# keith2018/TinyGPT

Hardware: AMD Instinct MI355X
Metric: decode tokens/sec (and % HBM roofline), Llama-3.2-1B bf16 batch=1, 1 GPU (higher is better)
Workload: dtype bf16; 1 GPU; Llama-3.2-1B bf16, batch 1 per GPU: 2048-token prefill then greedy decode (one step = one token, context 2054..3411); replicas=1, params=1235814400, graph=True

## Files before the change

tinygpt_amd/csrc/ctx.h:

```cpp
#pragma once
#include <hip/hip_runtime.h>

#include <algorithm>
#include <cmath>
#include <cstdarg>
#include <cstdio>
#include <cstdlib>
#include <cstring>
#include <string>
#include <vector>

#include "../../include/tgx.h"
#include "kernels/common.h"
#include "kv_pool.h"
#include "dev_mem.h"

using tgx::bf16_t;
typedef unsigned char ebyte;

namespace tgx { struct SampScratch; struct LpRecord; struct LpRow; }

constexpr int MAX_TICKET_EVENTS = 64;
constexpr int HOST_RING = 256;

struct PackedMat {
  unsigned char* P = nullptr;
  tgx::u32x4* rec = nullptr;
  long long row_bytes = 0;
  unsigned int base2 = 0;
  int ks = 0;
  int max_row_esc = 0;
  long long n_esc = 0;
};

struct LayerW {
  ebyte *in_norm = nullptr, *post_norm = nullptr;
  ebyte *wqkv = nullptr, *bqkv = nullptr, *wo = nullptr, *wgu = nullptr, *wdown = nullptr;
  PackedMat pgu, pdown;
  ebyte *q_norm = nullptr, *k_norm = nullptr;
  bool q_norm_ok = false, k_norm_ok = false;
  int merged_filled = 0;
  bool in_norm_ok = false, post_norm_ok = false, wo_ok = false, wdown_ok = false;
  ebyte *in_norm_b = nullptr, *post_norm_b = nullptr, *bo = nullptr, *bfc = nullptr, *bdown = nullptr;
  int gpt2_filled = 0;
};

struct RowState {
  float *x = nullptr, *q = nullptr, *attn = nullptr, *h = nullptr;
  float* k_raw = nullptr;
  float* logits = nullptr;
  float* probs = nullptr;
  float* part_val = nullptr;
  int* part_idx = nullptr;
  float* attn_part = nullptr;
  int *tok = nullptr, *pos = nullptr;
  long long* prompt = nullptr;
  ebyte *kcache = nullptr, *vcache = nullptr;
  const int* tbl = nullptr;
};

struct RowHost {
  int64_t past = 0;
  bool tok = false;
  bool idle = false;
  bool nologits = false;
  char fin = 0;
  int64_t lp_count = 0;
  bool probs_ok = false; tgx_sampler_cfg probs_cfg{};
  bool probs_proc = false;
  int auto_id = -1;
  void restart(int64_t len, bool idle_, char fin_) { past = len; tok = nologits = false; idle = idle_; fin = fin_; }
};

struct Tune {
  int ks = 1;
  int bpc = 4;
};

struct Profiler {
  bool on = false;
  hipEvent_t ev[2 * 8] = {};
  int64_t launches[TGX_KERNEL_COUNT] = {};
  double ms[TGX_KERNEL_COUNT] = {};
};

struct QkvEpi { bf16_t *q_hi = nullptr, *q_lo = nullptr, *k = nullptr, *v = nullptr; int past = 0; const int* tbl = nullptr; };

struct ScoreCall {
  int top_n = 0, n_score = 0;
  const long long* ids = nullptr;
  void* host = nullptr; size_t host_bytes = 0;
};

struct EmbedCall {
  static constexpr int SLICE = 32;
  int pool = 0, normalize = 0, dims = 0;
  int n = 0;
  int cur = 0;
  std::vector<int> tab;
  int slices = 0;
  float* host_out = nullptr;
  int np(int t) const { return tab[(size_t)t * 4 + 1]; }
};

namespace tgx { struct RgSeq; struct RgItem; struct MixItem; }
struct RaggedPass {
  int n = 0, M = 0, longest = 0;
  const int *rows = nullptr, *lens = nullptr, *first = nullptr;
  const long long* ids = nullptr;
  const tgx::RgSeq* seq = nullptr;
  const int* tok_seq = nullptr;
  const tgx::RgItem* items = nullptr;
  int n_items = 0;
  const int* past = nullptr;
  int ext_ns = 0;
  const tgx::MixItem *mix_split = nullptr, *mix_merge = nullptr;
  int n_mix_split = 0, n_mix_merge = 0, mix_slots = 0;
};

inline void* hip_dev_alloc(size_t bytes) { void* p = nullptr; return hipMalloc(&p, bytes) == hipSuccess ? p : nullptr; }
inline void hip_dev_free(void* p) { (void)hipFree(p); }
struct tgx_ctx {
  tgx_model_desc d{};
  DevMem mem{hip_dev_alloc, hip_dev_free};
  int device = 0;
  int num_cus = 256;
  hipStream_t stream = nullptr;
  std::string err;
  bool finalized = false;

  int dt = tgx::DT_BF16;
  size_t esz = 2;
  ebyte *embed = nullptr, *lm_head = nullptr, *final_norm = nullptr;
  ebyte *wpe = nullptr, *final_norm_b = nullptr;
  bool embed_ok = false, lm_head_ok = false, final_norm_ok = false, wpe_ok = false, final_norm_b_ok = false;
  bool gpt2 = false;
  std::vector<LayerW> L;
  int weights_packed = 1, packed_classes = 4, packed_matrices = 0, packed_fallbacks = 0, packed_max_row_esc = 0;
  PackedMat plm;
  float *rope_cos = nullptr, *rope_sin = nullptr;
  std::vector<RowState> rows;
  float *slab_x = nullptr, *slab_q = nullptr, *slab_kraw = nullptr, *slab_attn = nullptr, *slab_h = nullptr, *slab_logits = nullptr;
  float *slab_probs = nullptr, *slab_part_val = nullptr, *slab_attn_part = nullptr;
  int *slab_part_idx = nullptr, *slab_tok = nullptr, *slab_pos = nullptr;
  long long* slab_prompt = nullptr;
  ebyte *slab_k = nullptr, *slab_v = nullptr;
  size_t kv_row_elems = 0, attn_part_row = 0;
  RowState chunk[4];
  float *ch_x = nullptr, *ch_q = nullptr, *ch_kraw = nullptr, *ch_attn = nullptr, *ch_h = nullptr, *ch_part = nullptr;
  int* ch_pos = nullptr;

  int64_t past = 0;
  std::vector<RowHost> row_host;
  tgx::RowReq* row_req = nullptr;
  std::vector<tgx::RowReq> row_req_host;
  int row_union = -1;
  int batch = 0;
  bool have_logits = false, have_token = false;

  int* step = nullptr;
  int* step_done = nullptr;
  int* tok_log = nullptr;
  int log_cap = 0;
  int* host_ring = nullptr;
  int* host_ring_dev = nullptr;
  int64_t steps_issued = 0;
  hipEvent_t ticket_ev[MAX_TICKET_EVENTS] = {};
  int32_t last_sampled0 = -1;

  hipGraphExec_t step_graph = nullptr;
  hipGraphExec_t multi_graph = nullptr;
  struct GraphSet { hipGraphExec_t step = nullptr, multi = nullptr; int batch = 0; tgx_sampler_cfg cfg{}; int rows = -1; bool direct = false, mfma = false, nw4 = false; unsigned long long used = 0; };
  GraphSet graph_cache[6];
  unsigned long long graph_clock = 0;
  int graph_cur = -1;
  bool mirror_to_host = true;
  int graph_steps = 16;
  unsigned long long* seed_dev = nullptr;
  unsigned long long seed_on_dev = 0;
  bool seed_valid = false;
  tgx::SampScratch* samp_scratch = nullptr;
  unsigned long long* samp_list_comp = nullptr;
  float* samp_list_v = nullptr;
  bool have_probs = false;
  bool use_graph = true;

  Tune tune[TGX_KERNEL_COUNT];
  int lm_grid = 0, attn_nsplit = 1, attn_nsplit_opt = 0;
  int ws_rows = 0;
  float *ws_x = nullptr, *ws_out = nullptr;
  bf16_t *ws_ah = nullptr, *ws_al = nullptr;
  bf16_t* ws_al2 = nullptr;
  bf16_t *ws_qh = nullptr, *ws_ql = nullptr;
  bf16_t *ws_hh = nullptr, *ws_hl = nullptr;
  float* ws_part = nullptr; size_t ws_part_bytes = 0;
  bool poisoned = false;
  const char* launch_fault = nullptr;
  int* ws_pos = nullptr;
  float* ws_ssq = nullptr;
  int gemm_splitk = 1;
  int wide_n_min = 2;
  QkvEpi qkv_epi;
  int attn_dma = 1;
  int attn_ksplit = 1;
  int qk_fuse = 1;
  int prefill_skinny_hidden_max_wide = 2048;
  int prefill_skinny_rows = 128;
  int prefill_skinny_hidden_max = 8192;
  int skinny_dma = 1;
  int skinny_dma_rows = 1;
  int skinny_dma_oproj = 2;
  int skinny_dma_qkv = 2;
  int skinny_dma_nbw = 0;
  int decode_step_rows = 128;
  int prefill_skinny = 1;
  int skinny_wgs = 256;
  int skinny_gu_split = 0;
  int skinny_cfg_mid = 0;
  int skinny_cfg_force = -1;
  int decode_mfma_min = 3;
  bool prefill_mfma = true;
  int prefill_min_rows = 4;
  int prefill_f32_min_rows = 16;
  int gemm_tm = 0;
  int gemm_dma = 15 | (1 << 4) | (2 << 8);
  int wide_8k_max = 8;
  int debug_attn = 0;
  int attn_gmax = 0;
  int attn_direct_nw4 = 0;
  bool attn_nw4 = false;
  int attn_raw_fuse = 2;
  int attn_batch_nw8 = 1;
  int attn_batch_la = 0;
  int attn_batch_mfma = 17;
  int attn_direct_g = 1;
  int attn_direct_max = 384;
  bool attn_direct = false;
  int skinny_terms = 1;
  int skinny_ksplit = 1;
  int defer_min_rows = 129;
  int defer_reduce = 1;
  int attn_mfma_min = -1;
  bool attn_mfma = false;
  int debug_gemv = 0;
  int debug_skip = 0;
  int prof_same_layer = 0;
  int oproj_sliced = 1;
  int act16 = 0, act16_kernels = 1;
  int prefill_terms_rows = 16;
  int wide_8k_eff = 76;
  int skinny_terms_above = 2;
  int qkv_nosplit = 1;
  int splitk_8k = 1;
  bf16_t* ws_zero = nullptr;
  int oproj_fused = 1, attn_fused_max = 640, attn_fused_nw4 = 384;
  int kv_budget_tokens = 0;
  bool kv_paged = false;
  KvPool kv;
  int* kv_tbl = nullptr;
  long long* slab_acc = nullptr;
  unsigned char* rg_buf = nullptr; size_t rg_bytes = 0;
  float *rg_x = nullptr, *rg_logits = nullptr, *rg_part_val = nullptr; int* rg_part_idx = nullptr;
  int extend_attn_splits = -1;
  int extend_attn_min64 = 512, extend_attn_min128 = 1024;
  float* ext_part = nullptr; size_t ext_part_bytes = 0;
  enum { VERIFY_ROWS = TGX_MAX_DRAFT + 1 };
  float *vf_x = nullptr, *vf_logits = nullptr, *vf_part_val = nullptr; int *vf_part_idx = nullptr, *vf_rec = nullptr;
  int vf_pass_rows = 0;
  tgx::SampScratch* vs_scratch = nullptr;
  unsigned long long* vs_list_comp = nullptr;
  float* vs_list_v = nullptr;
  int* vs_draws = nullptr;
  enum { VERIFY_POSITIONS = TGX_MAX_VERIFY_POSITIONS };
  float *vj_x = nullptr, *vj_logits = nullptr, *vj_part_val = nullptr; int *vj_part_idx = nullptr, *vj_rec = nullptr, *vj_draws = nullptr;
  unsigned char* vj_args = nullptr;
  std::vector<unsigned char> vj_args_host;
  bool vf_pass_joint = false;
  int verify_last_form = 0, verify_last_splits = 0;
  int advance_attn_tiles = 16, advance_last_form = 0, advance_last_tiles = 0;
  float* mix_part = nullptr; size_t mix_part_bytes = 0;
  tgx::LpRecord* lp_ring = nullptr;
  tgx::LpRow* lp_rows = nullptr;
  float* lp_tile_max = nullptr;
  double* lp_tile_sum = nullptr;
  unsigned long long* lp_tile_keys = nullptr;
  int score_rows = 2048, score_vocab_chunk = 16384, score_last_form = 0;
  float* sc_logits = nullptr; size_t sc_logits_bytes = 0;
  unsigned char* sc_part = nullptr; size_t sc_part_bytes = 0;
  int sc_part_rows = 0;
  unsigned char* sc_out = nullptr; size_t sc_out_bytes = 0;
  unsigned char* em_buf = nullptr; size_t em_bytes = 0;
// ... 140 lines not shown
```

tinygpt_amd/csrc/decode.hip:

```cpp
#include "ctx.h"
#include "kernels/attn_decode.h"
#include "kernels/gemv.h"
#include "kernels/gemv_packed.h"
#include "kernels/oproj_sliced.h"
#include "kernels/verify.h"

int gemv_grid(const tgx_ctx* c, int units, int ks, int bpc) {
  const int upb = 4 / ks;
  const int want = (units + upb - 1) / upb;
  const int cap = c->num_cus * bpc;
  return want < cap ? want : cap;
}

static int gemv_nx(int K, int ks) { return ((K / 8) + ks * 64 - 1) / (ks * 64); }

static int gemv_auto_ks(int K, int want) {
  int ks = want;
  while (ks < 4 && gemv_nx(K, ks) > 8) ks *= 2;
  return ks;
}

static tgx::GemvArgs gemv_row(const tgx_ctx* c, tgx::GemvArgs a, int r) {
  a.x += (size_t)r * a.x_stride;
  if (a.out) a.out += (size_t)r * a.out_stride;
  if (a.q_out) a.q_out += (size_t)r * a.q_stride;
  if (a.k_raw) a.k_raw += (size_t)r * a.kraw_stride;
  if (a.k_cache) a.k_cache = (ebyte*)a.k_cache + (size_t)r * a.kv_stride * c->esz;
  if (a.v_cache) a.v_cache = (ebyte*)a.v_cache + (size_t)r * a.kv_stride * c->esz;
  if (a.pos) a.pos += r;
  if (a.blk_tbl) a.blk_tbl += (size_t)r * a.tbl_stride;
  if (a.logits) a.logits += (size_t)r * a.logits_stride;
  if (a.part_val) a.part_val += (size_t)r * a.part_stride;
  if (a.part_idx) a.part_idx += (size_t)r * a.part_stride;
  return a;
}

template <int DT, int PRO, int EPI, int NX>
static void launch_gemv_nx(tgx_ctx* c, const tgx::GemvArgs& a, int grid, int R) {
  const dim3 g(grid), b(256);
  if (R == 4) { hipLaunchKernelGGL((tgx::gemv_kernel<DT, PRO, EPI, NX, 4>), g, b, 0, c->stream, a); return; }
  if (R == 2) { hipLaunchKernelGGL((tgx::gemv_kernel<DT, PRO, EPI, NX, 2>), g, b, 0, c->stream, a); return; }
  if constexpr (DT != tgx::DT_F32 && ((PRO == tgx::PRO_RMSNORM && EPI == tgx::EPI_SILU_MUL) || (PRO == tgx::PRO_PLAIN && EPI == tgx::EPI_RESIDUAL))) {
    if (R == 1 && (a.x_acc || a.res_acc)) { hipLaunchKernelGGL((tgx::gemv_kernel<DT, PRO, EPI, NX, 1, true>), g, b, a.x_acc ? (size_t)a.K * 4 : 0, c->stream, a); return; }
  }
  for (int r = 0; r < R; r++) hipLaunchKernelGGL((tgx::gemv_kernel<DT, PRO, EPI, NX, 1>), g, b, 0, c->stream, gemv_row(c, a, r));
}

template <int PRO, int EPI, int NX>
static void launch_gemv_packed_nx(tgx_ctx* c, const tgx::GemvPackedArgs& p, int grid) {
  const dim3 g(grid), b(256);
  if constexpr (EPI != tgx::EPI_LOGITS) {
    if (p.g.x_acc || p.g.res_acc) { hipLaunchKernelGGL((tgx::gemv_packed_kernel<PRO, EPI, NX, true>), g, b, p.g.x_acc ? (size_t)p.g.K * 4 : 0, c->stream, p); return; }
  }
  hipLaunchKernelGGL((tgx::gemv_packed_kernel<PRO, EPI, NX, false>), g, b, 0, c->stream, p);
}

template <int PRO, int EPI>
static void launch_gemv_packed(tgx_ctx* c, const tgx::GemvArgs& a, const PackedMat& pk, int grid, int nx) {
  tgx::GemvPackedArgs p{};
  p.g = a; p.P = pk.P; p.rec = pk.rec; p.row_bytes = pk.row_bytes; p.base2 = pk.base2;
  switch (nx) {
    case 1: launch_gemv_packed_nx<PRO, EPI, 1>(c, p, grid); break;
    case 2: launch_gemv_packed_nx<PRO, EPI, 2>(c, p, grid); break;
    case 3: launch_gemv_packed_nx<PRO, EPI, 3>(c, p, grid); break;
    case 4: launch_gemv_packed_nx<PRO, EPI, 4>(c, p, grid); break;
    case 5: launch_gemv_packed_nx<PRO, EPI, 5>(c, p, grid); break;
    case 6: launch_gemv_packed_nx<PRO, EPI, 6>(c, p, grid); break;
    case 7: launch_gemv_packed_nx<PRO, EPI, 7>(c, p, grid); break;
    default: launch_gemv_packed_nx<PRO, EPI, 8>(c, p, grid); break;
  }
}

static int pack_matrix(tgx_ctx* c, const ebyte* W, int N, int K, int cls, int* stat_dev, PackedMat* out) {
  const int ks = gemv_auto_ks(K, c->tune[cls].ks), nx = gemv_nx(K, ks);
  if (K % 8 || K > tgx::PACKED_K_MAX || nx > 8) return TGX_OK;
  PackedMat m;
  m.ks = ks; m.row_bytes = (long long)ks * ((nx + 3) / 4) * 3072;
  int rc;
  if ((rc = dev_alloc(c, &m.P, (size_t)N * (size_t)m.row_bytes)) || (rc = dev_alloc(c, &m.rec, (size_t)N))) { dev_free(c, &m.P); return rc; }
  HIP_OK(c, hipMemsetAsync(stat_dev, 0, 4 * sizeof(int), c->stream));
  const size_t n8 = (size_t)N * K / 8;
  hipLaunchKernelGGL(tgx::packed_maxexp_kernel, dim3((unsigned)std::min<size_t>((n8 + 255) / 256, 4096)), dim3(256), 0, c->stream, reinterpret_cast<const bf16_t*>(W), n8, stat_dev);
  tgx::PackRowsArgs a{};
  a.W = reinterpret_cast<const bf16_t*>(W); a.N = N; a.K = K; a.ks = ks; a.nx = nx; a.P = m.P; a.rec = m.rec; a.row_bytes = m.row_bytes; a.stat = stat_dev;
  hipLaunchKernelGGL(tgx::pack_rows_kernel, dim3(N), dim3(64), 0, c->stream, a);
  int stat[4] = {0, 0, 0, 0};
  HIP_OK(c, hipGetLastError());
  HIP_OK(c, hipMemcpyAsync(stat, stat_dev, sizeof(stat), hipMemcpyDeviceToHost, c->stream));
  HIP_OK(c, hipStreamSynchronize(c->stream));
  c->packed_max_row_esc = std::max(c->packed_max_row_esc, stat[3]);
  if (stat[1] > 0) {
    dev_free(c, &m.P); dev_free(c, &m.rec);
    c->packed_fallbacks++;
    return TGX_OK;
  }
  const unsigned int E0 = (unsigned int)std::max(stat[0] - 15, 0);
  m.base2 = (E0 << 7) | (E0 << 23); m.n_esc = stat[2]; m.max_row_esc = stat[3];
  *out = m;
  c->packed_matrices++;
  return TGX_OK;
}

int pack_weights(tgx_ctx* c) {
  const tgx_model_desc& d = c->d;
  if (!c->weights_packed || c->dt != tgx::DT_BF16 || c->gpt2) return TGX_OK;
  int* stat_dev = nullptr;
  int rc = dev_alloc(c, &stat_dev, 4);
  for (size_t l = 0; l < c->L.size() && !rc; l++) {
    LayerW& w = c->L[l];
    if (c->packed_classes & 1) rc = pack_matrix(c, w.wgu, 2 * d.inter, d.hidden, TGX_KERNEL_GATEUP, stat_dev, &w.pgu);
    if (!rc && (c->packed_classes & 2) && d.inter <= 16384) rc = pack_matrix(c, w.wdown, d.hidden, d.inter, TGX_KERNEL_DOWN, stat_dev, &w.pdown);
  }
  if (!rc && (c->packed_classes & 4)) rc = pack_matrix(c, d.tied ? c->embed : c->lm_head, d.vocab, d.hidden, TGX_KERNEL_LMHEAD, stat_dev, &c->plm);
  dev_free(c, &stat_dev);
  return rc;
}

template <int PRO, int EPI>
static void launch_gemv(tgx_ctx* c, tgx::GemvArgs a, int cls, int R, const PackedMat* pk = nullptr) {
  const Tune& tn = c->tune[cls];
  a.dbg = ((c->debug_gemv >> (8 + cls)) & 1) ? (c->debug_gemv & 15) : 0;
  if (!a.ldw) a.ldw = a.K;
  a.ks = gemv_auto_ks(a.K, tn.ks);
  while (R > 1 && a.ks < 4 && gemv_nx(a.K, a.ks) > 4) a.ks *= 2;
  if (R == 2 && cls == TGX_KERNEL_GATEUP && a.ks == 1 && gemv_nx(a.K, 1) == 4) a.ks = 2;
  const int grid = (EPI == tgx::EPI_LOGITS) ? c->lm_grid : gemv_grid(c, a.units, a.ks, tn.bpc);
  const int nx = gemv_nx(a.K, a.ks);
  if constexpr ((PRO == tgx::PRO_RMSNORM && (EPI == tgx::EPI_SILU_MUL || EPI == tgx::EPI_LOGITS)) || (PRO == tgx::PRO_PLAIN && EPI == tgx::EPI_RESIDUAL)) {
    if (pk && pk->P && R == 1 && pk->ks == a.ks && a.ldw == a.K && !a.dbg) { launch_gemv_packed<PRO, EPI>(c, a, *pk, grid, nx); return; }
  }
  if constexpr (PRO == tgx::PRO_LAYERNORM || EPI == tgx::EPI_GELU) {
    TGX_DT_SWITCH(c->dt, switch (nx) {
      case 1: launch_gemv_nx<DT, PRO, EPI, 1>(c, a, grid, R); break;
      case 2: launch_gemv_nx<DT, PRO, EPI, 2>(c, a, grid, R); break;
      case 3: launch_gemv_nx<DT, PRO, EPI, 3>(c, a, grid, R); break;
      default: launch_gemv_nx<DT, PRO, EPI, 4>(c, a, grid, R); break;
    })
  } else {
    TGX_DT_SWITCH(c->dt, switch (nx) {
      case 1: launch_gemv_nx<DT, PRO, EPI, 1>(c, a, grid, R); break;
      case 2: launch_gemv_nx<DT, PRO, EPI, 2>(c, a, grid, R); break;
      case 3: launch_gemv_nx<DT, PRO, EPI, 3>(c, a, grid, R); break;
      case 4: launch_gemv_nx<DT, PRO, EPI, 4>(c, a, grid, R); break;
      case 5: launch_gemv_nx<DT, PRO, EPI, 5>(c, a, grid, R); break;
      case 6: launch_gemv_nx<DT, PRO, EPI, 6>(c, a, grid, R); break;
      case 7: launch_gemv_nx<DT, PRO, EPI, 7>(c, a, grid, R); break;
      default: launch_gemv_nx<DT, PRO, EPI, 8>(c, a, grid, R); break;
    })
  }
}

static void fill_strides(const tgx_ctx* c, tgx::GemvArgs& a) {
  const tgx_model_desc& d = c->d;
  a.x_stride = 0; a.out_stride = 0;
  a.q_stride = (long long)d.heads * d.head_dim; a.kraw_stride = (long long)d.kv_heads * d.head_dim;
  a.kv_stride = (long long)c->kv_row_elems; a.logits_stride = d.vocab; a.part_stride = c->lm_grid;
  a.act16 = c->act16;
}

static bool qk_fused(const tgx_ctx* c, long long kv_stride) { return c->d.qk_norm && c->d.head_dim == 128 && kv_stride != 0 && c->qk_fuse; }

bool oproj_sliced_ok(const tgx_ctx* c, int R, long long kv_stride) {
  const tgx_model_desc& d = c->d;
  if (!c->oproj_sliced || R != 1 || kv_stride == 0 || c->attn_direct || c->attn_mfma || c->gpt2 || c->dt == tgx::DT_F32 || !c->slab_acc) return false;
  if (d.head_dim != 64 || d.qk_norm || d.inter > 16384 || c->attn_nsplit > 32) return false;
  if (d.hidden > tgx::XACC_HIDDEN_MAX) return false;
  const int qd = d.heads * d.head_dim;
  if (qd % 256 == 0) return d.hidden % tgx::oproj_sliced_rows<32>() == 0;
  return qd % 128 == 0 && d.hidden % tgx::oproj_sliced_rows<16>() == 0;
}

bool oproj_fused_capable(const tgx_ctx* c) {
  const tgx_model_desc& d = c->d;
  if (!c->oproj_fused || c->gpt2 || c->dt == tgx::DT_F32 || !c->slab_acc) return false;
  return d.head_dim == 64 && !d.qk_norm && d.inter <= 16384 && d.hidden % 8 == 0 && d.hidden <= tgx::XACC_HIDDEN_MAX;
}
bool oproj_fused_ok(const tgx_ctx* c, int R, long long kv_stride) {
  return R == 1 && c->batch == 1 && kv_stride != 0 && c->attn_direct && oproj_fused_capable(c);
}
static bool resid_fixed(const tgx_ctx* c, int R, long long kv_stride) { return oproj_sliced_ok(c, R, kv_stride) || oproj_fused_ok(c, R, kv_stride); }

int launch_layer_kernel(tgx_ctx* c, RowState* rv, int R, int l, int cls, float* resid, long long kv_stride) {
  const tgx_model_desc& d = c->d;
  RowState& r = rv[0];
  const int H = d.hidden, I = d.inter, hd = d.head_dim, qd = d.heads * hd, kvd = d.kv_heads * hd;
  const size_t kv_layer = (c->kv_paged ? (size_t)c->kv.n_blocks() * d.kv_heads * tgx::KV_BLOCK : (size_t)d.kv_heads * d.max_ctx) * hd * c->esz;
  const long long kvs = c->kv_paged ? 0 : kv_stride, tbs = (c->kv_paged && kv_stride != 0) ? c->kv.tbl_stride() : 0;
  const LayerW& w = c->L[(size_t)l];
  switch (cls) {
    case TGX_KERNEL_QKV: {
      tgx::GemvArgs a{};
      fill_strides(c, a);
      a.W = w.wqkv; a.bias = w.bqkv; a.x = r.x; a.x_stride = H; a.norm_w = w.in_norm; a.eps = d.norm_eps;
      a.N = qd + 2 * kvd; a.K = H; a.units = a.N / 2;
      a.q_out = r.q; a.k_cache = r.kcache + (size_t)l * kv_layer; a.v_cache = r.vcache + (size_t)l * kv_layer; a.kv_stride = kvs;
      a.blk_tbl = r.tbl; a.tbl_stride = tbs;
      a.rope_cos = c->rope_cos; a.rope_sin = c->rope_sin; a.pos = r.pos;
      a.heads = d.heads; a.kv_heads = d.kv_heads; a.hd = hd; a.max_ctx = d.max_ctx;
      a.raw_qk = d.qk_norm ? 1 : 0; a.k_raw = r.k_raw;
      if (c->gpt2) {
        a.norm_b = w.in_norm_b;
        launch_gemv<tgx::PRO_LAYERNORM, tgx::EPI_QKV_ROPE>(c, a, TGX_KERNEL_QKV, R);
        break;
      }
      launch_gemv<tgx::PRO_RMSNORM, tgx::EPI_QKV_ROPE>(c, a, TGX_KERNEL_QKV, R);
      if (d.qk_norm && !qk_fused(c, kv_stride)) {
        tgx::QkNormArgs n{};
        n.q = r.q; n.k_raw = r.k_raw; n.k_cache = r.kcache + (size_t)l * kv_layer; n.q_norm_w = w.q_norm; n.k_norm_w = w.k_norm;
        n.rope_cos = c->rope_cos; n.rope_sin = c->rope_sin; n.pos = r.pos;
        n.heads = d.heads; n.kv_heads = d.kv_heads; n.hd = hd; n.max_ctx = d.max_ctx; n.eps = d.norm_eps;
        n.q_stride = qd; n.kraw_stride = kvd; n.kv_stride = kvs; n.blk_tbl = r.tbl; n.tbl_stride = tbs;
        TGX_DT_SWITCH(c->dt, hipLaunchKernelGGL(tgx::qk_norm_rope_kernel<DT>, dim3(d.heads + d.kv_heads, R), dim3(64), 0, c->stream, n))
      }
      break;
    }
    case TGX_KERNEL_ATTN: {
      tgx::AttnArgs a{};
      a.q = r.q; a.k_cache = r.kcache + (size_t)l * kv_layer; a.v_cache = r.vcache + (size_t)l * kv_layer;
      a.pos = r.pos; a.part = r.attn_part; a.out = r.attn;
      a.heads = d.heads; a.kv_heads = d.kv_heads; a.max_ctx = d.max_ctx; a.nsplit = c->attn_nsplit;
      a.scale = 1.0f / sqrtf((float)hd);
      a.q_stride = qd; a.kv_stride = kvs; a.part_stride = (long long)c->attn_part_row; a.dbg = c->debug_attn;
      a.blk_tbl = r.tbl; a.tbl_stride = tbs;
      a.act16 = c->act16 ? (c->dt == tgx::DT_BF16 ? 1 : (c->dt == tgx::DT_F16 ? 2 : 0)) : 0;
      if (qk_fused(c, kv_stride)) {
        a.k_raw = r.k_raw; a.kraw_stride = kvd; a.q_norm_w = w.q_norm; a.k_norm_w = w.k_norm;
        a.rope_cos = c->rope_cos; a.rope_sin = c->rope_sin; a.eps = d.norm_eps;
      }
      if (oproj_fused_ok(c, R, kv_stride)) {
        a.oj_w = w.wo; a.oj_x = r.x; a.oj_acc = c->slab_acc + (size_t)(&r - c->rows.data()) * H; a.oj_H = H; a.oj_ldw = qd;
      }
      launch_attn(c, a, R, !oproj_sliced_ok(c, R, kv_stride));
      break;
    }
    case TGX_KERNEL_OPROJ: {
      if (oproj_fused_ok(c, R, kv_stride)) return 0;
      tgx::GemvArgs a{};
      fill_strides(c, a);
      a.W = w.wo; a.bias = w.bo; a.x = r.attn; a.x_stride = qd; a.N = H; a.K = qd; a.units = (H + 1) / 2; a.out = resid; a.out_stride = H; a.hd = 2;
      if (oproj_sliced_ok(c, R, kv_stride)) {
        tgx::OprojSlicedArgs o{};
        o.W = w.wo; o.ldw = qd; o.part = r.attn_part; o.nsplit = c->attn_nsplit; o.x = r.x; o.acc = c->slab_acc + (size_t)(&r - c->rows.data()) * H; o.H = H; o.act16 = c->act16;
        const dim3 blk(256);
        TGX_DT16_SWITCH(c->dt,
          if (qd % 256 == 0) hipLaunchKernelGGL((tgx::oproj_sliced_kernel<DT, 64, 32>), dim3(H / tgx::oproj_sliced_rows<32>(), qd / 256), blk, 0, c->stream, o);
          else hipLaunchKernelGGL((tgx::oproj_sliced_kernel<DT, 64, 16>), dim3(H / tgx::oproj_sliced_rows<16>(), qd / 128), blk, 0, c->stream, o);)
        break;
      }
      launch_gemv<tgx::PRO_PLAIN, tgx::EPI_RESIDUAL>(c, a, TGX_KERNEL_OPROJ, R);
      break;
// ... 145 lines not shown
```

tinygpt_amd/csrc/kernels/gemv_packed.h:

```cpp
#pragma once
#include "gemv.h"

namespace tgx {

constexpr int PACKED_ESC = 4;
constexpr int PACKED_K_MAX = 32768;

struct PackedQuad { u32x4 s01, s23, c; };

struct GemvPackedArgs {
  GemvArgs g;
  const unsigned char* P;
  const u32x4* rec;
  long long row_bytes;
  unsigned int base2;
};

__device__ __forceinline__ bool packed_has_escape(unsigned int C) { return ((C - 0x11111111u) & ~C & 0x88888888u) != 0; }

__device__ __forceinline__ Slice8<DT_BF16> packed_decode(unsigned int S0, unsigned int S1, unsigned int C, unsigned int base2, const u32x4 rec, int chunk) {
  Slice8<DT_BF16> o;
  o.v[0] = ((S0 & 0x007f007fu) | ((S0 << 8) & 0x80008000u)) + ((( C        & 0x000f000fu) << 7) + base2);
  o.v[1] = (((S0 >> 8) & 0x007f007fu) | (S0 & 0x80008000u)) + ((((C >> 4)  & 0x000f000fu) << 7) + base2);
  o.v[2] = ((S1 & 0x007f007fu) | ((S1 << 8) & 0x80008000u)) + ((((C >> 8)  & 0x000f000fu) << 7) + base2);
  o.v[3] = (((S1 >> 8) & 0x007f007fu) | (S1 & 0x80008000u)) + ((((C >> 12) & 0x000f000fu) << 7) + base2);
  if (packed_has_escape(C)) {
#pragma unroll
    for (int e = 0; e < PACKED_ESC; e++) {
      const unsigned int en = rec[e];
      const unsigned int t = (en >> 16) & 7u, sh = (t & 1u) << 4;
      const unsigned int dsel = (en >> 19) == (unsigned int)chunk ? (t >> 1) : 4u;
      const unsigned int m = 0xffffu << sh, val = (en & 0xffffu) << sh;
#pragma unroll
      for (int dd = 0; dd < 4; dd++) o.v[dd] = dsel == (unsigned int)dd ? ((o.v[dd] & ~m) | val) : o.v[dd];
    }
  }
  return o;
}

template <int PRO, int EPI, int NX, bool XACC = false>
__global__ __launch_bounds__(256, NX <= 4 ? 4 : 1) void gemv_packed_kernel(const GemvPackedArgs pa) {
  constexpr int DT = DT_BF16;
  constexpr int NQ = (NX + 3) / 4;
  typedef elem_t<DT> E;
  static_assert(PRO == PRO_PLAIN || PRO == PRO_RMSNORM, "packed forms: plain or RMSNorm prologue");
  static_assert(EPI == EPI_SILU_MUL || EPI == EPI_RESIDUAL || EPI == EPI_LOGITS, "packed forms: gate_up, down, lm_head");
  const GemvArgs& a = pa.g;
  const int n_wg = (int)gridDim.x;
  __shared__ float ps[4][2];
  __shared__ float sv[1][4];
  __shared__ int si[1][4];

  const int lane = threadIdx.x & 63, wv = threadIdx.x >> 6;
  const int KS = a.ks, UPB = 4 / KS;
  const int slot = wv / KS, kpart = wv - slot * KS;
  const int nchunk = a.K >> 3;
  const int per = ((nchunk + KS * 64 - 1) / (KS * 64)) * 64;
  const int c_begin = min(kpart * per, nchunk), c_end = min(c_begin + per, nchunk);
  const int stride = n_wg * UPB;

  int cidx[NX];
  bool cok[NX];
#pragma unroll
  for (int j = 0; j < NX; j++) {
    const int c = c_begin + lane + 64 * j;
    cok[j] = c < c_end;
    cidx[j] = cok[j] ? c : max(c_end - 1, 0);
  }

  const size_t lane_off = (size_t)kpart * NQ * 3072 + (size_t)lane * 16;
  PackedQuad wa[NQ], wb[NQ], na[NQ], nb[NQ];
  u32x4 ea, eb, nea = {}, neb = {};
  auto load_unit = [&](int ub, PackedQuad* ta, PackedQuad* tb, u32x4& ra_rec, u32x4& rb_rec) {
    const int u = min(ub + slot, a.units - 1);
    int ra, rb; bool v;
    unit_rows<EPI>(a, u, ra, rb, v);
    ra_rec = pa.rec[ra]; rb_rec = pa.rec[rb];
    const unsigned char* pra = pa.P + (size_t)ra * pa.row_bytes + lane_off;
    const unsigned char* prb = pa.P + (size_t)rb * pa.row_bytes + lane_off;
#pragma unroll
    for (int q = 0; q < NQ; q++) {
      const u32x4* qa = reinterpret_cast<const u32x4*>(pra + (size_t)q * 3072);
      const u32x4* qb = reinterpret_cast<const u32x4*>(prb + (size_t)q * 3072);
      ta[q].s01 = load_nt(qa); ta[q].s23 = load_nt(qa + 64); ta[q].c = load_nt(qa + 128);
      tb[q].s01 = load_nt(qb); tb[q].s23 = load_nt(qb + 64); tb[q].c = load_nt(qb + 128);
    }
  };
  auto rec_uniform = [](const u32x4 v) {
    return u32x4{(unsigned int)__builtin_amdgcn_readfirstlane((int)v[0]), (unsigned int)__builtin_amdgcn_readfirstlane((int)v[1]),
                 (unsigned int)__builtin_amdgcn_readfirstlane((int)v[2]), (unsigned int)__builtin_amdgcn_readfirstlane((int)v[3])};
  };

  float xr[NX][8];
  auto load_x = [&]() {
    const f32x4* xg = reinterpret_cast<const f32x4*>(a.x);
#pragma unroll
    for (int j = 0; j < NX; j++) {
      f32x4 v0 = xg[2 * cidx[j]], v1 = xg[2 * cidx[j] + 1];
      if (!cok[j]) { v0 = f32x4{0.f, 0.f, 0.f, 0.f}; v1 = v0; }
#pragma unroll
      for (int t = 0; t < 4; t++) { xr[j][t] = v0[t]; xr[j][4 + t] = v1[t]; }
    }
  };
  ulonglong2 xacc0[(XACC && PRO == PRO_RMSNORM) ? 4 : 1];
  if constexpr (XACC && PRO == PRO_RMSNORM) {
    const ulonglong2* ag = reinterpret_cast<const ulonglong2*>(a.x_acc + (size_t)min((int)threadIdx.x, nchunk - 1) * 8);
#pragma unroll
    for (int q = 0; q < 4; q++) xacc0[q] = ag[q];
    __builtin_amdgcn_sched_barrier(0);
  }
  int ub = blockIdx.x * UPB;
  if (ub < a.units) load_unit(ub, wa, wb, nea, neb);
  Slice8<DT> nw_x[(XACC && PRO == PRO_RMSNORM) ? NX : 1];
  if constexpr (XACC && PRO == PRO_RMSNORM) {
#pragma unroll
    for (int j = 0; j < NX; j++) nw_x[j] = load_slice<DT>(static_cast<const E*>(a.norm_w), cidx[j]);
    __builtin_amdgcn_sched_barrier(0);
  }

  if constexpr (XACC && PRO == PRO_RMSNORM) {
    extern __shared__ __attribute__((aligned(16))) float xs[];
    for (int cs = threadIdx.x; cs < nchunk; cs += 256) {
      ulonglong2 t[4];
      if (cs == (int)threadIdx.x) {
#pragma unroll
        for (int q = 0; q < 4; q++) t[q] = xacc0[q];
      } else {
        const ulonglong2* ag = reinterpret_cast<const ulonglong2*>(a.x_acc + (size_t)cs * 8);
#pragma unroll
        for (int q = 0; q < 4; q++) t[q] = ag[q];
      }
      float f[8];
#pragma unroll
      for (int q = 0; q < 4; q++) { f[2 * q] = fix_to_f32((long long)t[q].x); f[2 * q + 1] = fix_to_f32((long long)t[q].y); }
      f32x4* dst = reinterpret_cast<f32x4*>(xs + (size_t)cs * 8);
      dst[0] = f32x4{f[0], f[1], f[2], f[3]}; dst[1] = f32x4{f[4], f[5], f[6], f[7]};
    }
    __syncthreads();
#pragma unroll
    for (int j = 0; j < NX; j++) {
      const f32x4* xl = reinterpret_cast<const f32x4*>(xs + (size_t)cidx[j] * 8);
      f32x4 v0 = xl[0], v1 = xl[1];
      if (!cok[j]) { v0 = f32x4{0.f, 0.f, 0.f, 0.f}; v1 = v0; }
#pragma unroll
      for (int t = 0; t < 4; t++) { xr[j][t] = v0[t]; xr[j][4 + t] = v1[t]; }
    }
  } else {
    load_x();
  }
  auto ks_sum = [&](float& v) {
    if (lane == 0) ps[wv][0] = v;
    __syncthreads();
    float t = ps[slot * KS][0];
    for (int k = 1; k < KS; k++) t += ps[slot * KS + k][0];
    v = t;
    __syncthreads();
  };
  if (PRO == PRO_RMSNORM) {
    const E* wg = static_cast<const E*>(a.norm_w);
    Slice8<DT> nw[NX];
#pragma unroll
    for (int j = 0; j < NX; j++) { if constexpr (XACC) nw[j] = nw_x[j]; else nw[j] = load_slice<DT>(wg, cidx[j]); }
    float ss = 0.f;
#pragma unroll
    for (int j = 0; j < NX; j++)
#pragma unroll
      for (int t = 0; t < 8; t++) ss = fmaf(xr[j][t], xr[j][t], ss);
    float ssq = wave_sum(ss);
    if (KS > 1) ks_sum(ssq);
    const float inv = 1.0f / sqrtf(ssq / (float)a.K + a.eps);
#pragma unroll
    for (int j = 0; j < NX; j++) {
      float w[8];
      slice_unpack<DT>(nw[j], w);
#pragma unroll
      for (int t = 0; t < 8; t++) xr[j][t] = w[t] * (xr[j][t] * inv);
    }
  }

  if constexpr (PRO != PRO_PLAIN) {
    if (a.act16) {
#pragma unroll
      for (int j = 0; j < NX; j++)
#pragma unroll
        for (int t = 0; t < 8; t++) xr[j][t] = elem_to_f32<DT>(f32_to_elem<DT>(xr[j][t]));
    }
  }

  float best_val = -INFINITY;
  int best_idx = 0x7fffffff;
  ea = rec_uniform(nea); eb = rec_uniform(neb);

  for (; ub < a.units; ub += stride) {
    const bool has_next = ub + stride < a.units;
    if (has_next) load_unit(ub + stride, na, nb, nea, neb);

    const int u = ub + slot;
    const bool writer = u < a.units && kpart == 0 && lane == 0;
    int ra = 0, rb = 0; bool rb_valid = false;
    float e0 = 0.f, e1 = 0.f;
    if (writer) {
      unit_rows<EPI>(a, u, ra, rb, rb_valid);
      if (EPI == EPI_RESIDUAL) {
        if constexpr (XACC) { e0 = fix_to_f32(a.res_acc[ra]); e1 = fix_to_f32(a.res_acc[rb]); }
        else { e0 = a.out[ra]; e1 = a.out[rb]; }
      }
    }

    float acc_a0 = 0.f, acc_b0 = 0.f, acc_a1 = 0.f, acc_b1 = 0.f;
#pragma unroll
    for (int j = 0; j < NX; j++) {
      const f32x4 xa = f32x4{xr[j][0], xr[j][1], xr[j][2], xr[j][3]};
      const f32x4 xb = f32x4{xr[j][4], xr[j][5], xr[j][6], xr[j][7]};
      const int q = j >> 2, jj = j & 3;
      const u32x4 sa4 = (jj & 2) ? wa[q].s23 : wa[q].s01, sb4 = (jj & 2) ? wb[q].s23 : wb[q].s01;
      const int chunk = c_begin + lane + 64 * j;
      const Slice8<DT> da = packed_decode(sa4[(jj & 1) * 2], sa4[(jj & 1) * 2 + 1], wa[q].c[jj], pa.base2, ea, chunk);
      const Slice8<DT> db = packed_decode(sb4[(jj & 1) * 2], sb4[(jj & 1) * 2 + 1], wb[q].c[jj], pa.base2, eb, chunk);
      if (j & 1) { acc_a1 = dot8<DT>(acc_a1, da, xa, xb); acc_b1 = dot8<DT>(acc_b1, db, xa, xb); }
      else       { acc_a0 = dot8<DT>(acc_a0, da, xa, xb); acc_b0 = dot8<DT>(acc_b0, db, xa, xb); }
    }
    float sa = wave_sum(acc_a0 + acc_a1);
    float sb = wave_sum(acc_b0 + acc_b1);

    if (KS > 1) {
      __syncthreads();
      if (lane == 0) { ps[wv][0] = sa; ps[wv][1] = sb; }
      __syncthreads();
      if (kpart == 0) {
        sa = ps[slot * KS][0]; sb = ps[slot * KS][1];
        for (int k = 1; k < KS; k++) { sa += ps[slot * KS + k][0]; sb += ps[slot * KS + k][1]; }
      }
    }

    if (writer) {
      float va = sa, vb = sb;
      if (EPI == EPI_LOGITS) {
        a.logits[ra] = va;
        if (va > best_val) { best_val = va; best_idx = ra; }
        if (rb_valid) {
          a.logits[rb] = vb;
          if (vb > best_val) { best_val = vb; best_idx = rb; }
        }
      } else {
        if (a.bias) { const E* bias = static_cast<const E*>(a.bias); va += elem_to_f32<DT>(bias[ra]); vb += elem_to_f32<DT>(bias[rb]); }
        if (EPI == EPI_RESIDUAL) {
          a.out[ra] = e0 + va;
          if (rb_valid) a.out[rb] = e1 + vb;
          if constexpr (XACC) { a.res_acc[ra] = 0; if (rb_valid) a.res_acc[rb] = 0; }
        } else if (EPI == EPI_SILU_MUL) {
          a.out[u] = round_storage_if<DT>((va / (1.0f + expf(-va))) * vb, a.act16);
        }
      }
    }

#pragma unroll
    for (int q = 0; q < NQ; q++) { wa[q] = na[q]; wb[q] = nb[q]; }
    ea = rec_uniform(nea); eb = rec_uniform(neb);
  }

  if (EPI == EPI_LOGITS) {
    if (lane == 0) { sv[0][wv] = best_val; si[0][wv] = best_idx; }
    __syncthreads();
    if (threadIdx.x == 0) {
      float bv = sv[0][0]; int bi = si[0][0];
      for (int w = 1; w < 4; w++)
        if (sv[0][w] > bv || (sv[0][w] == bv && si[0][w] < bi)) { bv = sv[0][w]; bi = si[0][w]; }
      a.part_val[blockIdx.x] = bv;
      a.part_idx[blockIdx.x] = bi;
    }
  }
}

__global__ __launch_bounds__(256) void packed_maxexp_kernel(const bf16_t* W, size_t n8, int* stat) {
  int m = 0;
  for (size_t i = (size_t)blockIdx.x * 256 + threadIdx.x; i < n8; i += (size_t)gridDim.x * 256) {
    const u32x4 v = reinterpret_cast<const u32x4*>(W)[i];
#pragma unroll
    for (int t = 0; t < 4; t++) {
      const int e0 = (v[t] >> 7) & 0xff, e1 = (v[t] >> 23) & 0xff;
      if (e0 < 255) m = max(m, e0);
      if (e1 < 255) m = max(m, e1);
    }
  }
#pragma unroll
  for (int o = 32; o > 0; o >>= 1) m = max(m, __shfl_xor(m, o, 64));
  if ((threadIdx.x & 63) == 0) atomicMax(stat, m);
}

struct PackRowsArgs {
  const bf16_t* W;
  int N, K, ks, nx;
  unsigned char* P;
  u32x4* rec;
  long long row_bytes;
  int* stat;
};

__global__ __launch_bounds__(64) void pack_rows_kernel(const PackRowsArgs a) {
  __shared__ unsigned int ent[PACKED_ESC];
  const int row = blockIdx.x, lane = threadIdx.x;
  const int E0 = max(a.stat[0] - 15, 0);
  const bf16_t* w = a.W + (size_t)row * a.K;
  if (lane < PACKED_ESC) ent[lane] = 0xffffffffu;
  __syncthreads();
  int cnt = 0;
  for (int k0 = 0; k0 < a.K; k0 += 64) {
    const int k = k0 + lane;
    unsigned int bits = 0; bool esc = false;
    if (k < a.K) { bits = w[k]; const int code = (int)((bits >> 7) & 0xff) - E0; esc = code < 1 || code > 15; }
    const unsigned long long bal = __ballot(esc);
    const int p = cnt + __popcll(bal & ((1ull << lane) - 1ull));
    if (esc && p < PACKED_ESC) ent[p] = ((unsigned int)k << 16) | bits;
    cnt += __popcll(bal);
  }
  __syncthreads();
  if (lane == 0) {
    a.rec[row] = u32x4{ent[0], ent[1], ent[2], ent[3]};
    if (cnt > PACKED_ESC) atomicAdd(a.stat + 1, 1);
    if (cnt) { atomicAdd(a.stat + 2, cnt); atomicMax(a.stat + 3, cnt); }
  }
  const int nchunk = a.K >> 3, nq = (a.nx + 3) / 4;
  const int per = ((nchunk + a.ks * 64 - 1) / (a.ks * 64)) * 64;
  for (int p = 0; p < a.ks; p++) {
    const int c_begin = min(p * per, nchunk), c_end = min(c_begin + per, nchunk);
    for (int q = 0; q < nq; q++) {
      unsigned int S[8], C[4];
#pragma unroll
      for (int jj = 0; jj < 4; jj++) {
        const int j = 4 * q + jj, c = c_begin + lane + 64 * j;
        S[2 * jj] = 0; S[2 * jj + 1] = 0; C[jj] = 0x11111111u;
        if (j < a.nx && c < c_end) {
          const u32x4 v = reinterpret_cast<const u32x4*>(w)[c];
          unsigned int b[8], cd[8];
#pragma unroll
          for (int t = 0; t < 8; t++) {
            const unsigned int bits = (v[t >> 1] >> (16 * (t & 1))) & 0xffffu;
            const int code = (int)((bits >> 7) & 0xff) - E0;
            b[t] = ((bits >> 8) & 0x80u) | (bits & 0x7fu);
            cd[t] = (code < 1 || code > 15) ? 0u : (unsigned int)code;
          }
          S[2 * jj] = b[0] | (b[2] << 8) | (b[1] << 16) | (b[3] << 24);
          S[2 * jj + 1] = b[4] | (b[6] << 8) | (b[5] << 16) | (b[7] << 24);
          unsigned int cc = 0;
#pragma unroll
          for (int t = 0; t < 4; t++) cc |= (cd[2 * t] << (4 * t)) | (cd[2 * t + 1] << (4 * t + 16));
          C[jj] = cc;
        }
      }
      u32x4* dst = reinterpret_cast<u32x4*>(a.P + (size_t)row * a.row_bytes + ((size_t)p * nq + q) * 3072) + lane;
      dst[0] = u32x4{S[0], S[1], S[2], S[3]};
      dst[64] = u32x4{S[4], S[5], S[6], S[7]};
      dst[128] = u32x4{C[0], C[1], C[2], C[3]};
    }
  }
}

}
```

Measured before the change: 1556 tokens/s.

## Repack 12-bit weight encoding into byte-aligned high/low halves with perm-based decode

```diff
diff --git a/tinygpt_amd/csrc/ctx.h b/tinygpt_amd/csrc/ctx.h
--- a/tinygpt_amd/csrc/ctx.h
+++ b/tinygpt_amd/csrc/ctx.h
@@ -27,7 +27,7 @@
   unsigned char* P = nullptr;
   tgx::u32x4* rec = nullptr;
   long long row_bytes = 0;
-  unsigned int base2 = 0;
+  unsigned int e0h4 = 0;
   int ks = 0;
   int max_row_esc = 0;
   long long n_esc = 0;
@@ -136,7 +136,7 @@
   bool embed_ok = false, lm_head_ok = false, final_norm_ok = false, wpe_ok = false, final_norm_b_ok = false;
   bool gpt2 = false;
   std::vector<LayerW> L;
-  int weights_packed = 1, packed_classes = 4, packed_matrices = 0, packed_fallbacks = 0, packed_max_row_esc = 0;
+  int weights_packed = 1, packed_classes = 5, packed_matrices = 0, packed_fallbacks = 0, packed_max_row_esc = 0;
   PackedMat plm;
   float *rope_cos = nullptr, *rope_sin = nullptr;
   std::vector<RowState> rows;
diff --git a/tinygpt_amd/csrc/decode.hip b/tinygpt_amd/csrc/decode.hip
--- a/tinygpt_amd/csrc/decode.hip
+++ b/tinygpt_amd/csrc/decode.hip
@@ -58,7 +58,7 @@
 template <int PRO, int EPI>
 static void launch_gemv_packed(tgx_ctx* c, const tgx::GemvArgs& a, const PackedMat& pk, int grid, int nx) {
   tgx::GemvPackedArgs p{};
-  p.g = a; p.P = pk.P; p.rec = pk.rec; p.row_bytes = pk.row_bytes; p.base2 = pk.base2;
+  p.g = a; p.P = pk.P; p.rec = pk.rec; p.row_bytes = pk.row_bytes; p.e0h4 = pk.e0h4;
   switch (nx) {
     case 1: launch_gemv_packed_nx<PRO, EPI, 1>(c, p, grid); break;
     case 2: launch_gemv_packed_nx<PRO, EPI, 2>(c, p, grid); break;
@@ -94,8 +94,8 @@
     c->packed_fallbacks++;
     return TGX_OK;
   }
-  const unsigned int E0 = (unsigned int)std::max(stat[0] - 15, 0);
-  m.base2 = (E0 << 7) | (E0 << 23); m.n_esc = stat[2]; m.max_row_esc = stat[3];
+  const unsigned int E0h = (unsigned int)std::max((stat[0] >> 1) - 7, 0);
+  m.e0h4 = E0h * 0x01010101u; m.n_esc = stat[2]; m.max_row_esc = stat[3];
   *out = m;
   c->packed_matrices++;
   return TGX_OK;
diff --git a/tinygpt_amd/csrc/kernels/gemv_packed.h b/tinygpt_amd/csrc/kernels/gemv_packed.h
--- a/tinygpt_amd/csrc/kernels/gemv_packed.h
+++ b/tinygpt_amd/csrc/kernels/gemv_packed.h
@@ -6,36 +6,52 @@
 constexpr int PACKED_ESC = 4;
 constexpr int PACKED_K_MAX = 32768;
 
-struct PackedQuad { u32x4 s01, s23, c; };
+struct PackedQuad { u32x4 l01, l23, nb; };
 
 struct GemvPackedArgs {
   GemvArgs g;
   const unsigned char* P;
   const u32x4* rec;
   long long row_bytes;
-  unsigned int base2;
+  unsigned int e0h4;
 };
 
-__device__ __forceinline__ bool packed_has_escape(unsigned int C) { return ((C - 0x11111111u) & ~C & 0x88888888u) != 0; }
-
-__device__ __forceinline__ Slice8<DT_BF16> packed_decode(unsigned int S0, unsigned int S1, unsigned int C, unsigned int base2, const u32x4 rec, int chunk) {
-  Slice8<DT_BF16> o;
-  o.v[0] = ((S0 & 0x007f007fu) | ((S0 << 8) & 0x80008000u)) + ((( C        & 0x000f000fu) << 7) + base2);
-  o.v[1] = (((S0 >> 8) & 0x007f007fu) | (S0 & 0x80008000u)) + ((((C >> 4)  & 0x000f000fu) << 7) + base2);
-  o.v[2] = ((S1 & 0x007f007fu) | ((S1 << 8) & 0x80008000u)) + ((((C >> 8)  & 0x000f000fu) << 7) + base2);
-  o.v[3] = (((S1 >> 8) & 0x007f007fu) | (S1 & 0x80008000u)) + ((((C >> 12) & 0x000f000fu) << 7) + base2);
-  if (packed_has_escape(C)) {
-#pragma unroll
-    for (int e = 0; e < PACKED_ESC; e++) {
-      const unsigned int en = rec[e];
-      const unsigned int t = (en >> 16) & 7u, sh = (t & 1u) << 4;
-      const unsigned int dsel = (en >> 19) == (unsigned int)chunk ? (t >> 1) : 4u;
-      const unsigned int m = 0xffffu << sh, val = (en & 0xffffu) << sh;
-#pragma unroll
-      for (int dd = 0; dd < 4; dd++) o.v[dd] = dsel == (unsigned int)dd ? ((o.v[dd] & ~m) | val) : o.v[dd];
-    }
-  }
-  return o;
+typedef float f32x2 __attribute__((ext_vector_type(2)));
+
+__device__ __forceinline__ f32x2 pk_fma_x0(f32x2 w, f32x2 x, f32x2 acc) {
+  asm("v_pk_fma_f32 %0, %1, %2, %0 op_sel_hi:[1,0,1]" : "+v"(acc) : "v"(w), "v"(x));
+  return acc;
+}
+__device__ __forceinline__ f32x2 pk_fma_x1(f32x2 w, f32x2 x, f32x2 acc) {
+  asm("v_pk_fma_f32 %0, %1, %2, %0 op_sel:[0,1,0] op_sel_hi:[1,1,1]" : "+v"(acc) : "v"(w), "v"(x));
+  return acc;
+}
+
+__device__ __forceinline__ unsigned int packed_high4(unsigned int t, unsigned int e0h4) { return (((t << 4) + t) & 0x87878787u) + e0h4; }
+template <int T> __device__ __forceinline__ float packed_weight(unsigned int H, unsigned int L) {
+  return __uint_as_float(__builtin_amdgcn_perm(H, L, ((4u + T) << 24) | ((unsigned int)T << 16) | 0x0c0cu));
+}
+struct PackedBytes { unsigned int H0, H1, L0, L1; };
+__device__ __forceinline__ PackedBytes packed_expand(unsigned int L0, unsigned int L1, unsigned int Nb, unsigned int e0h4) {
+  return PackedBytes{packed_high4(Nb & 0x0f0f0f0fu, e0h4), packed_high4((Nb >> 4) & 0x0f0f0f0fu, e0h4), L0, L1};
+}
+__device__ __forceinline__ void packed_weights(const PackedBytes& b, float f[8]) {
+  f[0] = packed_weight<0>(b.H0, b.L0); f[1] = packed_weight<1>(b.H0, b.L0); f[2] = packed_weight<2>(b.H0, b.L0); f[3] = packed_weight<3>(b.H0, b.L0);
+  f[4] = packed_weight<0>(b.H1, b.L1); f[5] = packed_weight<1>(b.H1, b.L1); f[6] = packed_weight<2>(b.H1, b.L1); f[7] = packed_weight<3>(b.H1, b.L1);
+}
+__device__ __forceinline__ void packed_repair(PackedBytes& b, const u32x4 rec, int c0, int lane) {
+#pragma unroll
+  for (int e = 0; e < PACKED_ESC; e++) {
+    const unsigned int en = rec[e], l = (en >> 19) - (unsigned int)c0;
+    if (l < 64u) {
+      const unsigned int sh = (en >> 13) & 0x18u;
+      const unsigned int vh = ((en >> 8) & 0xffu) << sh, vl = (en & 0xffu) << sh;
+      const unsigned int m = (unsigned int)lane == l ? 0xffu << sh : 0u;
+      const unsigned int m0 = (en & 0x40000u) ? 0u : m, m1 = (en & 0x40000u) ? m : 0u;
+      b.H0 = (b.H0 & ~m0) | (vh & m0); b.L0 = (b.L0 & ~m0) | (vl & m0);
+      b.H1 = (b.H1 & ~m1) | (vh & m1); b.L1 = (b.L1 & ~m1) | (vl & m1);
+    }
+  }
 }
 
 template <int PRO, int EPI, int NX, bool XACC = false>
@@ -58,6 +74,7 @@
   const int per = ((nchunk + KS * 64 - 1) / (KS * 64)) * 64;
   const int c_begin = min(kpart * per, nchunk), c_end = min(c_begin + per, nchunk);
   const int stride = n_wg * UPB;
+  const int c0_u = __builtin_amdgcn_readfirstlane(c_begin);
 
   int cidx[NX];
   bool cok[NX];
@@ -82,8 +99,8 @@
     for (int q = 0; q < NQ; q++) {
       const u32x4* qa = reinterpret_cast<const u32x4*>(pra + (size_t)q * 3072);
       const u32x4* qb = reinterpret_cast<const u32x4*>(prb + (size_t)q * 3072);
-      ta[q].s01 = load_nt(qa); ta[q].s23 = load_nt(qa + 64); ta[q].c = load_nt(qa + 128);
-      tb[q].s01 = load_nt(qb); tb[q].s23 = load_nt(qb + 64); tb[q].c = load_nt(qb + 128);
+      ta[q].l01 = load_nt(qa); ta[q].l23 = load_nt(qa + 64); ta[q].nb = load_nt(qa + 128);
+      tb[q].l01 = load_nt(qb); tb[q].l23 = load_nt(qb + 64); tb[q].nb = load_nt(qb + 128);
     }
   };
   auto rec_uniform = [](const u32x4 v) {
@@ -207,21 +224,29 @@
       }
     }
 
-    float acc_a0 = 0.f, acc_b0 = 0.f, acc_a1 = 0.f, acc_b1 = 0.f;
+    f32x2 acc0 = {0.f, 0.f}, acc1 = {0.f, 0.f};
+    const bool rep_a = ea[0] != 0xffffffffu, rep_b = eb[0] != 0xffffffffu;
 #pragma unroll
     for (int j = 0; j < NX; j++) {
-      const f32x4 xa = f32x4{xr[j][0], xr[j][1], xr[j][2], xr[j][3]};
-      const f32x4 xb = f32x4{xr[j][4], xr[j][5], xr[j][6], xr[j][7]};
       const int q = j >> 2, jj = j & 3;
-      const u32x4 sa4 = (jj & 2) ? wa[q].s23 : wa[q].s01, sb4 = (jj & 2) ? wb[q].s23 : wb[q].s01;
-      const int chunk = c_begin + lane + 64 * j;
-      const Slice8<DT> da = packed_decode(sa4[(jj & 1) * 2], sa4[(jj & 1) * 2 + 1], wa[q].c[jj], pa.base2, ea, chunk);
-      const Slice8<DT> db = packed_decode(sb4[(jj & 1) * 2], sb4[(jj & 1) * 2 + 1], wb[q].c[jj], pa.base2, eb, chunk);
-      if (j & 1) { acc_a1 = dot8<DT>(acc_a1, da, xa, xb); acc_b1 = dot8<DT>(acc_b1, db, xa, xb); }
-      else       { acc_a0 = dot8<DT>(acc_a0, da, xa, xb); acc_b0 = dot8<DT>(acc_b0, db, xa, xb); }
-    }
-    float sa = wave_sum(acc_a0 + acc_a1);
-    float sb = wave_sum(acc_b0 + acc_b1);
+      const u32x4 la4 = (jj & 2) ? wa[q].l23 : wa[q].l01, lb4 = (jj & 2) ? wb[q].l23 : wb[q].l01;
+      PackedBytes ba = packed_expand(la4[(jj & 1) * 2], la4[(jj & 1) * 2 + 1], wa[q].nb[jj], pa.e0h4);
+      PackedBytes bb = packed_expand(lb4[(jj & 1) * 2], lb4[(jj & 1) * 2 + 1], wb[q].nb[jj], pa.e0h4);
+      if (rep_a) packed_repair(ba, ea, c0_u + 64 * j, lane);
+      if (rep_b) packed_repair(bb, eb, c0_u + 64 * j, lane);
+      float fa[8], fb[8];
+      packed_weights(ba, fa); packed_weights(bb, fb);
+      f32x2 acc = (j & 1) ? acc1 : acc0;
+#pragma unroll
+      for (int t = 0; t < 8; t += 2) {
+        const f32x2 x2 = f32x2{xr[j][t], xr[j][t + 1]};
+        acc = pk_fma_x0(f32x2{fa[t], fb[t]}, x2, acc);
+        acc = pk_fma_x1(f32x2{fa[t + 1], fb[t + 1]}, x2, acc);
+      }
+      if (j & 1) acc1 = acc; else acc0 = acc;
+    }
+    float sa = wave_sum(acc0[0] + acc1[0]);
+    float sb = wave_sum(acc0[1] + acc1[1]);
 
     if (KS > 1) {
       __syncthreads();
@@ -288,6 +313,11 @@
   if ((threadIdx.x & 63) == 0) atomicMax(stat, m);
 }
 
+__device__ __forceinline__ bool packed_is_escape(unsigned int bits, int E0h) {
+  const int e = (int)((bits >> 7) & 0xff), d = (e >> 1) - E0h;
+  return d < 0 || d > 7 || e == 0 || e == 255;
+}
+
 struct PackRowsArgs {
   const bf16_t* W;
   int N, K, ks, nx;
@@ -300,7 +330,7 @@
 __global__ __launch_bounds__(64) void pack_rows_kernel(const PackRowsArgs a) {
   __shared__ unsigned int ent[PACKED_ESC];
   const int row = blockIdx.x, lane = threadIdx.x;
-  const int E0 = max(a.stat[0] - 15, 0);
+  const int E0h = max((a.stat[0] >> 1) - 7, 0);
   const bf16_t* w = a.W + (size_t)row * a.K;
   if (lane < PACKED_ESC) ent[lane] = 0xffffffffu;
   __syncthreads();
@@ -308,7 +338,7 @@
   for (int k0 = 0; k0 < a.K; k0 += 64) {
     const int k = k0 + lane;
     unsigned int bits = 0; bool esc = false;
-    if (k < a.K) { bits = w[k]; const int code = (int)((bits >> 7) & 0xff) - E0; esc = code < 1 || code > 15; }
+    if (k < a.K) { bits = w[k]; esc = packed_is_escape(bits, E0h); }
     const unsigned long long bal = __ballot(esc);
     const int p = cnt + __popcll(bal & ((1ull << lane) - 1ull));
     if (esc && p < PACKED_ESC) ent[p] = ((unsigned int)k << 16) | bits;
@@ -325,35 +355,35 @@
   for (int p = 0; p < a.ks; p++) {
     const int c_begin = min(p * per, nchunk), c_end = min(c_begin + per, nchunk);
     for (int q = 0; q < nq; q++) {
-      unsigned int S[8], C[4];
+      unsigned int L[8], Nb[4];
 #pragma unroll
       for (int jj = 0; jj < 4; jj++) {
         const int j = 4 * q + jj, c = c_begin + lane + 64 * j;
-        S[2 * jj] = 0; S[2 * jj + 1] = 0; C[jj] = 0x11111111u;
+        L[2 * jj] = 0; L[2 * jj + 1] = 0; Nb[jj] = 0;
         if (j < a.nx && c < c_end) {
           const u32x4 v = reinterpret_cast<const u32x4*>(w)[c];
-          unsigned int b[8], cd[8];
+          unsigned int lo[8], n[8];
 #pragma unroll
           for (int t = 0; t < 8; t++) {
             const unsigned int bits = (v[t >> 1] >> (16 * (t & 1))) & 0xffffu;
-            const int code = (int)((bits >> 7) & 0xff) - E0;
-            b[t] = ((bits >> 8) & 0x80u) | (bits & 0x7fu);
-            cd[t] = (code < 1 || code > 15) ? 0u : (unsigned int)code;
+            const bool esc = packed_is_escape(bits, E0h);
+            lo[t] = esc ? 0u : (bits & 0xffu);
+            n[t] = esc ? 0u : (((bits >> 12) & 8u) | (((bits >> 8) & 0x7fu) - (unsigned int)E0h));
           }
-          S[2 * jj] = b[0] | (b[2] << 8) | (b[1] << 16) | (b[3] << 24);
-          S[2 * jj + 1] = b[4] | (b[6] << 8) | (b[5] << 16) | (b[7] << 24);
-          unsigned int cc = 0;
-#pragma unroll
-          for (int t = 0; t < 4; t++) cc |= (cd[2 * t] << (4 * t)) | (cd[2 * t + 1] << (4 * t + 16));
-          C[jj] = cc;
+          L[2 * jj] = lo[0] | (lo[1] << 8) | (lo[2] << 16) | (lo[3] << 24);
+          L[2 * jj + 1] = lo[4] | (lo[5] << 8) | (lo[6] << 16) | (lo[7] << 24);
+          unsigned int nn = 0;
+#pragma unroll
+          for (int t = 0; t < 4; t++) nn |= (n[t] << (8 * t)) | (n[4 + t] << (8 * t + 4));
+          Nb[jj] = nn;
         }
       }
       u32x4* dst = reinterpret_cast<u32x4*>(a.P + (size_t)row * a.row_bytes + ((size_t)p * nq + q) * 3072) + lane;
-      dst[0] = u32x4{S[0], S[1], S[2], S[3]};
-      dst[64] = u32x4{S[4], S[5], S[6], S[7]};
-      dst[128] = u32x4{C[0], C[1], C[2], C[3]};
-    }
-  }
-}
-
-}
+      dst[0] = u32x4{L[0], L[1], L[2], L[3]};
+      dst[64] = u32x4{L[4], L[5], L[6], L[7]};
+      dst[128] = u32x4{Nb[0], Nb[1], Nb[2], Nb[3]};
+    }
+  }
+}
+
+}
```

Result: faster. 1577 tokens/s (median of 6 runs) (+1.4%).
